# hy-vision-learning/jck-generation

Hardware: AMD Instinct MI355X
Metric: images/sec (G+D step) DCGAN 64x64 bs256 (higher is better)
Workload: dtype bf16; 1 GPU; DCGAN 64x64x3 synthetic, batch 256 per GPU, full G+D step incl. GP pass, RNG and Adam (BASELINE.json configs[1]); per_gpu_batch=256, global_batch=256, parallelism=dp1, dead_D_wgrad_in_G_phase=skipped (never observable: zeroed at train/dcgan_trainer.py:155)

## Files before the change

include/jckgan.h:

```cpp
#ifndef JCKGAN_H
#define JCKGAN_H
#include <stddef.h>
#include <stdint.h>
#ifdef __cplusplus
extern "C" {
#endif

#define JCK_PREC_BF16 0
#define JCK_PREC_F32 1
#define JCK_PREC_BF16X3 2

#define JCK_OK 0
#define JCK_E_ARG (-1)
#define JCK_E_HIP (-2)
#define JCK_E_WS (-3)

const char* jck_last_error(void);
const char* jck_last_launch(void);
const char* jck_launch_name(int i);
int jck_version(void);
int jck_pad_rows(int c);
int jck_pad_chan(int c);

size_t jck_packed_bytes(int prec, long long elems);
// ... 48 lines not shown
                   float* dgamma, float* dbeta, long long rows, int C, void* stream);
int jck_bn_finalize_grouped(const float* stats, int slots_per_group, float count, const float* gamma, const float* beta, float eps,
                            float* aux, float* stat_out, int C, int groups, void* stream);
int jck_bn_fwd(int prec, const void* y, const float* stats, int slots_per_group, float count, const float* gamma, const float* beta,
               float eps, float slope, void* a, float* aux, float* stat_out, float* running_mean, float* running_var, int64_t* nbt,
               float momentum, long long rows_per_group, int C, int groups, void* stream);
int jck_bn_act_fwd_grouped(int prec, const void* y, const float* aux, float slope, void* a, long long rows_per_group, int C,
                           int groups, void* stream);
int jck_bn_act_bwd_grouped(int prec, const void* g_a, const void* y, const float* aux, float slope, float* sums, void* g_y,
                           float* dgamma, float* dbeta, long long rows_per_group, int C, int groups, int grad_groups, void* stream);
size_t jck_grid_sync_bytes(void);
int jck_grid_sync_error(const void* sync_ws);
int jck_bn_act_bwd_res(int prec, const void* g_a, const void* y, const float* aux, float slope, float* sums, void* g_y,
                       float* dgamma, float* dbeta, long long rows_per_group, int C, int groups, int grad_groups, void* sync_ws,
                       void* stream);
int jck_conv_down_grouped(int prec, const void* big, const void* w, void* small_out, float* stats, int* stats_slots, int N, int Hb,
                          int Wb, int Cb, int Cs, int group_images, void* stream);
int jck_conv_up_grouped(int prec, const void* small_in, const void* w, void* big_out, float* stats, int* stats_slots, int N, int Hs,
                        int Ws, int Cs, int Cb, int group_images, void* stream);
int jck_img_prep(int prec, const float* img_nchw, const float* noise_nchw, float keep, float mix, void* out, int N, int HW,
                 void* stream);
int jck_img_prep_u8(int prec, const unsigned char* data, const int64_t* idx, const float* noise, float keep, float mix,
                    void* out_nhwc4, float* out_nchw, int B, int Hs, int Ws, void* stream);
#define JCK_RESIZE_MAX_SRC 1024
#define JCK_RESIZE_TAPS_MAGIC 0x7a736572
long long jck_resize_taps_bytes(int Hs, int Ws, int S);
int jck_resize_taps_build(int Hs, int Ws, int S, void* host_buf);
int jck_img_prep_u8_any(int prec, const unsigned char* data, const int64_t* idx, const unsigned char* flip, const float* noise,
                        const unsigned* rng, int tensor_id, float keep, float mix, void* out_nhwc4, float* out_nchw, int B, int Hs,
                        int Ws, int S, const void* taps_dev, void* stream);
// ... 219 lines not shown
```

jck-generation_amd/csrc/engine.hip:

```cpp
#include <cstdlib>

#include "engine_internal.hpp"
#define JCK_BATCHED_DEFAULT 3

namespace {

constexpr long long ALIGN_F = 64;

void add_param(NetLayout& L, const char* name, int a, int b, int c, int d) {
  TensorInfo ti{name, 0, L.n_params, (long long)a * b * c * d, {a, b, c, d}};
  L.t.push_back(ti);
  L.n_params = (L.n_params + ti.numel + ALIGN_F - 1) / ALIGN_F * ALIGN_F;
}
void add_bn(NetLayout& L, const char* wn, const char* bn, const char* rm, const char* rv, int c) {
  add_param(L, wn, c, 1, 1, 1);
  add_param(L, bn, c, 1, 1, 1);
  TensorInfo m{rm, 1, L.n_bn, c, {c, 1, 1, 1}};
  L.t.push_back(m);
  L.n_bn += (c + ALIGN_F - 1) / ALIGN_F * ALIGN_F;
  TensorInfo v{rv, 2, L.n_bn, c, {c, 1, 1, 1}};
  L.t.push_back(v);
  L.n_bn += (c + ALIGN_F - 1) / ALIGN_F * ALIGN_F;
}

// ... 353 lines not shown
                                    e->P(e->LD, e->dg, "label_embedding.weight"), e->P(e->LD, e->dg, "label_embedding.bias"), B, ws));
  if (side) HIPCHK(hipEventRecord(e->evHead, side));
  return jck_split_rows(e->prec, e->gc, L1_KPAD, TT.FEAT, ga4_out, R3, st);
}

struct XgradEpi { const void* tanh_y; float scale; void* out; hipEvent_t done; bool fused; };
struct DBackward {
  int gw = 1;
  hipStream_t side = nullptr;
  bool join = true, lazy_join = false;
  int part = 0;
  bool resident = true;
  bool xgrad = false;
  XgradEpi* xe = nullptr;
  bool gp_norm = false;
};
static int d_convs_backward(jck_engine* e, const DActs& S, const void* x_in, int B, hipStream_t st, const DBackward& o) {
  const int G = S.groups, gw = o.gw;
  hipStream_t side = gw > 0 ? o.side : nullptr;
  for (int i = TT.NS - 1; i >= 0; --i) {
    const int hb = TT.D_HB[i], cs = TT.D_CS[i], cb = TT.D_CB[i];
    const long long rows = (long long)B * (hb / 2) * (hb / 2);
    const bool resume = o.part == 2 && i == TT.NS - 1;
    const bool split0 = !resume && i == 0 && e->bn_res && e->prec == JCK_PREC_BF16 && gw > 0 && gw < G;
    hipEvent_t done = side && e->ext_events && !resume ? e->evW[i] : nullptr;
    if (!resume)
      JCK_TRY(bn_act_bwd_res_ev(e->prec, S.g[i], S.y[i], S.aux[i], LRELU, S.sums[i], S.g[i], gw ? e->P(e->LD, e->dg, NWN[i]) : nullptr,
                                gw ? e->P(e->LD, e->dg, NBN[i]) : nullptr, rows, cs, split0 ? gw : G, gw,
                                e->bn_res && o.resident ? e->gsync : nullptr, st, done));
    if (!resume && gw) {
      hipStream_t ws;
      JCK_TRY(fork_side(e, i, st, side, &ws, !done));
      JCK_TRY(jck_conv_wgrad(e->prec, S.g[i], i == 0 ? x_in : S.a[i - 1], e->wg_ws, e->wg_ws_bytes, e->P(e->LD, e->dg, CWN[i]), 1, gw * B, hb, hb, cb,
                             cs, ws));
    }
    if (split0) {
      const DActs P = S.group(e, gw, G - gw);
      JCK_TRY(bn_act_bwd_res_ev(e->prec, P.g[i], P.y[i], P.aux[i], LRELU, P.sums[i], P.g[i], nullptr, nullptr, rows, cs, G - gw, 0, e->gsync, st, nullptr));
    }
    if (o.part == 1) {
      HIPCHK(hipEventRecord(e->evTail, side ? side : st));
      e->ss.tail_on_side = side != nullptr;
      if (side && !o.lazy_join) HIPCHK(hipStreamWaitEvent(st, e->evTail, 0));
      return JCK_OK;
    }
    if (i > 0)
      JCK_TRY(jck_conv_up(e->prec, S.g[i], e->d_up[i], S.g[i - 1], nullptr, nullptr, 0, G * B, hb / 2, hb / 2, cs, cb, st));
    else if (o.xgrad) {
      const void* g0 = S.group(e, G - 1, 1).g[0];
      if (o.xe) JCK_TRY(conv_up_tanh_bwd_ev(e->prec, g0, e->d_up[0], o.xe->tanh_y, o.xe->scale, o.xe->out, B, hb / 2, hb / 2, cs, cb, st, o.xe->done, &o.xe->fused));
      if (!o.xe || !o.xe->fused) JCK_TRY(jck_conv_up(e->prec, g0, e->d_up[0], S.gx, nullptr, nullptr, 0, B, hb / 2, hb / 2, cs, cb, st));
    }
  }
  if (o.gp_norm) JCK_TRY(jck_gp_norm(e->prec, S.gx, B, TT.HW, e->acc, 6, e->acc_ld, S.norms, st));
  if (side && o.join) {
    HIPCHK(hipEventRecord(e->evWdone, side));
    if (o.lazy_join) { e->ss.join_pending = true; e->ss.mid_recorded = false; }
    else HIPCHK(hipStreamWaitEvent(st, e->evWdone, 0));
  }
  return JCK_OK;
}
static int d_backward(jck_engine* e, DActs& D, const void* x_in, int B, const float* drop_mask, hipStream_t st, const DBackward& o,
                      bool head_mid_done = false) {
// ... 444 lines not shown
  return jck_engine_repack(e, 1, c.st);
}

static int phase_g_loss(jck_engine* e, const PhaseCtx& c) {
  JCK_TRY(clear_or_memset(e, e->ss.gg_clean_step, c.in->step, c.st, e->gg, e->LG.n_params * sizeof(float)));
  const bool fuse = e->head_fuse;
  JCK_TRY(d_forward(e, c.D0, e->fake, c.B, 3, c.in->drop_mask[3], c.st, !fuse));
  if (fuse && !c.cg) JCK_TRY(d_head(e, c.D0, c.B, 0.9f, 0, 2, 5, c.st, c.D0.g[TT.NS - 1]));
  else if (fuse) {
    const float tg1 = 0.9f;
    const int md1 = 0, sl1 = 2, sp1 = 5;
    JCK_TRY(cg_head_middle(e, c.B, 1, &tg1, &md1, &sl1, &sp1, c.D0.prob, c.D0.ds, c.in->drop_mask[3], c.st));
  } else JCK_TRY(d_head(e, c.D0, c.B, 0.9f, 0, 2, 5, c.st));
  XgradEpi xe = {e->fake_raw, 0.9f, e->g_raw, (c.sA && e->ext_events) ? e->evW[TT.NS - 1] : nullptr, false};
  DBackward bw;
  bw.gw = 0; bw.xgrad = true; bw.xe = e->fuse_tanh ? &xe : nullptr;
  JCK_TRY(d_backward(e, c.D0, e->fake, c.B, c.in->drop_mask[3], c.st, bw, fuse));
  return g_backward(e, c.D0.gx, c.B, c.st, c.sA, xe.fused);
}

static int phase_g_step(jck_engine* e, const PhaseCtx& c) {
  if (!e->hp_holds(c.in->step, c.in->lr) && !e->capturing) JCK_TRY(refresh_adam_scalars(e, c.in->step, c.in->lr, c.st));
  JCK_TRY(adam_net(e, 0, 0, e->LG.n_params, c.in->grad_scale, e->hp2 + 8 * e->parity, c.st, nullptr, e->gema));
  TailJobs t = {};
  for (int i = 0; i < TT.NS; ++i) {
    const int cs = TT.D_CS[i];
    t.l[i].rec = e->d_rs[i] + (size_t)e->parity * 4 * 2 * cs;
    t.l[i].rm = e->dbn + find(e->LD, RMN[i])->offset;
    t.l[i].rv = e->dbn + find(e->LD, RVN[i])->offset;
    t.l[i].nbt = (long long*)(e->dnbt + i);
    t.l[i].C = cs;
// ... 234 lines not shown
```

jck-generation_amd/csrc/ops.hip:

```cpp
#include "ops_internal.hpp"
#include "ew.hpp"
#include "ew_optim.hpp"
#include "latent.hpp"
#include "resize.hpp"

#include <cstdlib>
#include <cstring>
#include <string>

static thread_local std::string g_err;
void jck_set_error(const std::string& s) { g_err = s; }
extern "C" const char* jck_last_error(void) { return g_err.c_str(); }
#ifndef JCK_BUILD_ID
#define JCK_BUILD_ID 100
#endif
extern "C" int jck_version(void) { return JCK_BUILD_ID; }

struct KernelInfo { const char* launch; const char* label; };
#define SAME(s) {s, s}
static constexpr KernelInfo KERNELS[] = {
    SAME("igemm<bf16,128,128>"),   SAME("igemm<bf16,128,64>"),   SAME("igemm<bf16,64,128,img>"),   {nullptr, "igemm<bf16,64,128>"}, SAME("igemm<bf16,16,256>"),
    SAME("igemm<f32,128,128>"),    SAME("igemm<f32,128,64>"),    SAME("igemm<f32,64,128,img>"),    SAME("igemm<f32,64,128>"),       SAME("igemm<f32,16,256>"),
    SAME("igemm<bf16x3,128,128>"), SAME("igemm<bf16x3,128,64>"), SAME("igemm<bf16x3,64,128,img>"), SAME("igemm<bf16x3,64,128>"),    SAME("igemm<bf16x3,16,256>"),
    {"igemm_dma_persist<128,256,8>", "igemm<bf16,128,256>"}, {"igemm_dma_persist<128,128,4>", "igemm<bf16,128,128>"},
    {"igemm_dma_persist<128,64,4>", "igemm<bf16,128,64>"},   {"igemm_dma_persist<64,128,4>", "igemm<bf16,64,128>"},
    {"igemm_dma<128,256,3,ws,8>", "igemm<bf16,128,256>"},    {"igemm_dma<128,128,2>", "igemm<bf16,128,128>"},
    {"igemm_dma<128,64,3,ws>", "igemm<bf16,128,64>"},        {"igemm_dma<64,128,2>", "igemm<bf16,64,128>"},
    {"img_down", "img_down<bf16>"}, {"img_up", "img_up<bf16>"},
    {"wgrad_dma<3,ws>", "wgrad<bf16,128,128>"}, {"wgrad_dma<2>", "wgrad<bf16,128,128>"},
    SAME("wgrad<bf16,128,128>"),   SAME("wgrad<bf16,128,64>"),   SAME("wgrad<bf16,64,64,img>"),   SAME("wgrad<bf16,64,64>"),
    SAME("wgrad<f32,128,128>"),    SAME("wgrad<f32,128,64>"),    SAME("wgrad<f32,64,64,img>"),    SAME("wgrad<f32,64,64>"),
    SAME("wgrad<bf16x3,128,128>"), SAME("wgrad<bf16x3,128,64>"), SAME("wgrad<bf16x3,64,64,img>"), SAME("wgrad<bf16x3,64,64>"),
    {nullptr, "bn_act_fwd"}, {nullptr, "bn_bwd_resident"}, {nullptr, "bn_bwd_3launch"},
    {nullptr, "latent_loss"}, {nullptr, "latent_adam"},
    {nullptr, "conv_up_mask"}, {nullptr, "leaky_affine_bwd"}, {nullptr, "critic_ds"}, {nullptr, "latent_loss_ex"},
    {nullptr, "feat_match"}, {nullptr, "img_prep_u8_any"}};
#undef SAME
static_assert(sizeof(KERNELS) / sizeof(KERNELS[0]) == K_COUNT, "KERNELS and the KernelId offsets disagree");
constexpr bool same_str(const char* a, const char* b) { return *a == *b && (!*a || same_str(a + 1, b + 1)); }
constexpr bool row(KernelId id, const char* launch, const char* label) { return same_str(KERNELS[id].launch, launch) && same_str(KERNELS[id].label, label); }
static_assert(row(kid_igemm<PrecBf16, 128, 128, 1>(), "igemm<bf16,128,128>", "igemm<bf16,128,128>") && row(kid_igemm<PrecBf16, 128, 64, 1>(), "igemm<bf16,128,64>", "igemm<bf16,128,64>") && row(kid_igemm<PrecBf16, 64, 128, 2>(), "igemm<bf16,64,128,img>", "igemm<bf16,64,128,img>") && row(kid_igemm<PrecBf16, 16, 256, 1>(), "igemm<bf16,16,256>", "igemm<bf16,16,256>") &&
              row(kid_igemm<PrecF32, 128, 128, 1>(), "igemm<f32,128,128>", "igemm<f32,128,128>") && row(kid_igemm<PrecF32, 128, 64, 1>(), "igemm<f32,128,64>", "igemm<f32,128,64>") && row(kid_igemm<PrecF32, 64, 128, 2>(), "igemm<f32,64,128,img>", "igemm<f32,64,128,img>") && row(kid_igemm<PrecF32, 64, 128, 1>(), "igemm<f32,64,128>", "igemm<f32,64,128>") && row(kid_igemm<PrecF32, 16, 256, 1>(), "igemm<f32,16,256>", "igemm<f32,16,256>") &&
              row(kid_igemm<PrecBf16x3, 128, 128, 1>(), "igemm<bf16x3,128,128>", "igemm<bf16x3,128,128>") && row(kid_igemm<PrecBf16x3, 128, 64, 1>(), "igemm<bf16x3,128,64>", "igemm<bf16x3,128,64>") && row(kid_igemm<PrecBf16x3, 64, 128, 2>(), "igemm<bf16x3,64,128,img>", "igemm<bf16x3,64,128,img>") && row(kid_igemm<PrecBf16x3, 64, 128, 1>(), "igemm<bf16x3,64,128>", "igemm<bf16x3,64,128>") && row(kid_igemm<PrecBf16x3, 16, 256, 1>(), "igemm<bf16x3,16,256>", "igemm<bf16x3,16,256>") &&
              row(kid_igemm_dma(K_IGEMM_PERSIST, 128, 256), "igemm_dma_persist<128,256,8>", "igemm<bf16,128,256>") && row(kid_igemm_dma(K_IGEMM_PERSIST, 128, 128), "igemm_dma_persist<128,128,4>", "igemm<bf16,128,128>") && row(kid_igemm_dma(K_IGEMM_PERSIST, 128, 64), "igemm_dma_persist<128,64,4>", "igemm<bf16,128,64>") && row(kid_igemm_dma(K_IGEMM_PERSIST, 64, 128), "igemm_dma_persist<64,128,4>", "igemm<bf16,64,128>") &&
              row(kid_igemm_dma(K_IGEMM_DMA, 128, 256), "igemm_dma<128,256,3,ws,8>", "igemm<bf16,128,256>") && row(kid_igemm_dma(K_IGEMM_DMA, 128, 128), "igemm_dma<128,128,2>", "igemm<bf16,128,128>") && row(kid_igemm_dma(K_IGEMM_DMA, 128, 64), "igemm_dma<128,64,3,ws>", "igemm<bf16,128,64>") && row(kid_igemm_dma(K_IGEMM_DMA, 64, 128), "igemm_dma<64,128,2>", "igemm<bf16,64,128>") &&
              row(K_IMG_DOWN, "img_down", "img_down<bf16>") && row(K_IMG_UP, "img_up", "img_up<bf16>") && row(K_WGRAD_DMA_WS, "wgrad_dma<3,ws>", "wgrad<bf16,128,128>") && row(K_WGRAD_DMA, "wgrad_dma<2>", "wgrad<bf16,128,128>") &&
              row(kid_wgrad<PrecBf16, 128, 128, 1>(), "wgrad<bf16,128,128>", "wgrad<bf16,128,128>") && row(kid_wgrad<PrecBf16, 128, 64, 1>(), "wgrad<bf16,128,64>", "wgrad<bf16,128,64>") && row(kid_wgrad<PrecBf16, 64, 64, 2>(), "wgrad<bf16,64,64,img>", "wgrad<bf16,64,64,img>") && row(kid_wgrad<PrecBf16, 64, 64, 1>(), "wgrad<bf16,64,64>", "wgrad<bf16,64,64>") &&
              row(kid_wgrad<PrecF32, 128, 128, 1>(), "wgrad<f32,128,128>", "wgrad<f32,128,128>") && row(kid_wgrad<PrecF32, 128, 64, 1>(), "wgrad<f32,128,64>", "wgrad<f32,128,64>") && row(kid_wgrad<PrecF32, 64, 64, 2>(), "wgrad<f32,64,64,img>", "wgrad<f32,64,64,img>") && row(kid_wgrad<PrecF32, 64, 64, 1>(), "wgrad<f32,64,64>", "wgrad<f32,64,64>") &&
              row(kid_wgrad<PrecBf16x3, 128, 128, 1>(), "wgrad<bf16x3,128,128>", "wgrad<bf16x3,128,128>") && row(kid_wgrad<PrecBf16x3, 128, 64, 1>(), "wgrad<bf16x3,128,64>", "wgrad<bf16x3,128,64>") && row(kid_wgrad<PrecBf16x3, 64, 64, 2>(), "wgrad<bf16x3,64,64,img>", "wgrad<bf16x3,64,64,img>") && row(kid_wgrad<PrecBf16x3, 64, 64, 1>(), "wgrad<bf16x3,64,64>", "wgrad<bf16x3,64,64>") &&
              same_str(KERNELS[K_LATENT_LOSS].label, "latent_loss") && same_str(KERNELS[K_LATENT_ADAM].label, "latent_adam") &&
              same_str(KERNELS[K_CONV_UP_MASK].label, "conv_up_mask") && same_str(KERNELS[K_LEAKY_AFFINE_BWD].label, "leaky_affine_bwd") &&
              same_str(KERNELS[K_CRITIC_DS].label, "critic_ds") && same_str(KERNELS[K_LATENT_LOSS_EX].label, "latent_loss_ex") && same_str(KERNELS[K_FEAT_MATCH].label, "feat_match") && same_str(KERNELS[K_IMG_PREP_ANY].label, "img_prep_u8_any") &&
              same_str(KERNELS[K_BN_ACT_FWD].label, "bn_act_fwd") && same_str(KERNELS[K_BN_BWD_RES].label, "bn_bwd_resident") && same_str(KERNELS[K_BN_BWD_3L].label, "bn_bwd_3launch") &&
              kid_igemm<PrecBf16, 16, 256, 0>() == kid_igemm<PrecBf16, 16, 256, 1>() && !KERNELS[K_IGEMM + 3].launch,
              "KERNELS and the kid_* functions disagree");
static thread_local const char* g_last_launch = "";
void note_launch(KernelId k) { g_last_launch = KERNELS[k].launch ? KERNELS[k].launch : ""; }
extern "C" const char* jck_last_launch(void) { return g_last_launch; }
extern "C" const char* jck_launch_name(int i) {
  for (int k = 0; k < K_COUNT; ++k)
    if (KERNELS[k].launch && i-- == 0) return KERNELS[k].launch;
  return nullptr;
}
extern "C" int jck_pad_rows(int c) { return c <= 16 ? 16 : (c <= 64 ? 64 : (c + 127) / 128 * 128); }
extern "C" int jck_pad_chan(int c) { return c == 3 ? 4 : c; }

static int env_int(const char* name, int dflt) { const char* v = getenv(name); return v ? atoi(v) : dflt; }
// ... 712 lines not shown
```

jck-generation_amd/csrc/ops_bn.hip:

```cpp
#include "ops_internal.hpp"
#include "bn2.hpp"
#include "bnres.hpp"

#include <climits>

static bool bn_channels_ok(int C, int max_c = INT_MAX) { return is_pow2(C) && C >= 8 && C <= max_c; }

constexpr int BN_FUSE_WGS = 256;
static unsigned bn_slice_grid(long long rows, int C, int groups) {
  const long long per = std::max<long long>(1, BN_FUSE_WGS / ((long long)(C / 64) * groups));
  return (unsigned)std::max<long long>(1, std::min<long long>((rows + 31) / 32, per));
}
static bool bn_two_launches(int prec, int C) { return g_bn_bwd_fuse && C >= 64 && C % 64 == 0 && (prec == JCK_PREC_BF16 || g_bn_bwd_fuse > 1); }

extern "C" int jck_bn_finalize(const float* stats, int slots, float count, const float* gamma, const float* beta,
                               float* running_mean, float* running_var, int64_t* nbt, float momentum, float eps, float* aux,
                               int C, void* stream) {
  if (slots < 1) JCK_FAIL(JCK_E_ARG, "bn_finalize: slots must be >= 1");
  if (C % 4) JCK_FAIL(JCK_E_ARG, "bn_finalize: C % 4 != 0");
  hipLaunchKernelGGL(bn_finalize_kernel, dim3(C / 4), dim3(256), 0, (hipStream_t)stream, stats, slots, count, gamma, beta,
                     running_mean, running_var, (long long*)nbt, momentum, eps, aux, C);
  HIPCHK(hipGetLastError());
  return JCK_OK;
}
// ... 185 lines not shown
  const dim3 grid(nb), block(BNRES_THREADS);
  ProfScope prof(K_BN_BWD_RES, 0.0, stream, 3.0 * groups * rows_per_group * C * 2);
  const int ng = (groups >= 3 && 3 * nch <= 16) ? 3 : (groups >= 2 && 2 * nch <= 16) ? 2 : 1;
#define BNRES_CASE(NCH_, NG_) case NCH_ * 4 + NG_: LAUNCH_EV((bn_bwd_res_kernel<NCH_, NG_>), grid, block, 0, stream, done, p); break
  switch (nch * 4 + ng) {
    BNRES_CASE(1, 1); BNRES_CASE(2, 1); BNRES_CASE(4, 1); BNRES_CASE(8, 1); BNRES_CASE(16, 1);
    BNRES_CASE(1, 2); BNRES_CASE(2, 2); BNRES_CASE(4, 2); BNRES_CASE(8, 2);
    BNRES_CASE(1, 3); BNRES_CASE(2, 3); BNRES_CASE(4, 3);
    default: JCK_FAIL(JCK_E_ARG, "bn_act_bwd_res: no kernel for this plan");
  }
#undef BNRES_CASE
  HIPCHK(hipGetLastError());
  return JCK_OK;
}

extern "C" size_t jck_bn2_ws_floats(int C) { return (size_t)(4 + 4 * BN_BWD_MAX_BLOCKS) * C; }
extern "C" int jck_bn2_vchain(int prec, const void* v, const void* y, const void* gy, const float* aux, const float* s1,
                              const float* gamma, float slope, float* ws, void* u, void* xdir, float* dgamma, long long rows, int C,
                              void* stream) {
  if (!bn_channels_ok(C, 2048)) JCK_FAIL(JCK_E_ARG, "bn2_vchain: C must be a power of two in [8, 2048]");
  const int rstep = 256 / (C / 8);
  const int blocks = bn_bwd_blocks(rows, rstep);
  float* partial = ws + 4 * C;
  DISPATCH_T(prec, hipLaunchKernelGGL((bn2_reduce_kernel<T, 1>), dim3(blocks), dim3(256), 3 * C * rstep * sizeof(float),
                                      (hipStream_t)stream, (const T*)v, (const T*)y, (const T*)gy, aux, slope, partial, rows, C));
  HIPCHK(hipGetLastError());
  if (bn_two_launches(prec, C)) {
    DISPATCH_T(prec, hipLaunchKernelGGL(bn2_vchain_apply_fused_kernel<T>, dim3(bn_slice_grid(rows, C, 1), C / 64), dim3(BNF_THREADS), 0,
                                        (hipStream_t)stream, (const T*)v, (const T*)y, (const T*)gy, aux, s1, (const float*)partial, blocks, ws,
                                        gamma, dgamma, slope, 1.0f / (float)rows, (T*)u, (T*)xdir, rows, C));
// ... 42 lines not shown
```

jck-generation_amd/csrc/ops_internal.hpp:

```cpp
#pragma once
#include <hip/hip_ext.h>

#include <algorithm>
#include <cmath>
#include <string>

#include "../../include/jckgan.h"
#include "common.hpp"

void jck_set_error(const std::string& s);

static inline bool prec_f32_storage(int prec) { return prec == JCK_PREC_F32 || prec == JCK_PREC_BF16X3; }
static inline bool is_pow2(int v) { return v > 0 && (v & (v - 1)) == 0; }
static inline unsigned ew_grid(long long n, int per_block = 256) { return (unsigned)std::max<long long>(1, std::min<long long>((n + per_block - 1) / per_block, 8192)); }

#define JCK_FAIL(code, msg)                                   \
  do {                                                        \
    jck_set_error(std::string(__func__) + ": " + (msg));     \
    return (code);                                            \
  } while (0)

#define HIPCHK(expr)                                                                                     \
  do {                                                                                                   \
    hipError_t e_ = (expr);                                                                              \
// ... 25 lines not shown
  K_PRECS = 3,
  K_IGEMM_TILES = 5,
  K_DMA_TILES = 4,
  K_WGRAD_TILES = 4,
  K_IGEMM = 0,
  K_IGEMM_PERSIST = K_IGEMM + K_PRECS * K_IGEMM_TILES,
  K_IGEMM_DMA = K_IGEMM_PERSIST + K_DMA_TILES,
  K_IMG_DOWN = K_IGEMM_DMA + K_DMA_TILES, K_IMG_UP,
  K_WGRAD_DMA_WS, K_WGRAD_DMA,
  K_WGRAD,
  K_BN_ACT_FWD = K_WGRAD + K_PRECS * K_WGRAD_TILES, K_BN_BWD_RES, K_BN_BWD_3L,
  K_LATENT_LOSS, K_LATENT_ADAM,
  K_CONV_UP_MASK, K_LEAKY_AFFINE_BWD, K_CRITIC_DS, K_LATENT_LOSS_EX,
  K_FEAT_MATCH,
  K_IMG_PREP_ANY,
  K_COUNT
};
template <class P> constexpr int kid_prec() { return P::SPLIT ? 2 : P::IS_F32 ? 1 : 0; }
template <class P, int BCH, int BPIX, int NSUB> constexpr KernelId kid_igemm() {
  static_assert(P::IS_F32 || !(BCH == 64 && NSUB == 1), "bf16 has no register-staged 64 x 128 tile (and no name for one)");
  return KernelId(K_IGEMM + K_IGEMM_TILES * kid_prec<P>() + (BCH == 128 ? (BPIX == 128 ? 0 : 1) : BCH == 64 ? (NSUB == 2 ? 2 : 3) : 4));
}
constexpr KernelId kid_igemm_dma(KernelId family, int BCH, int BPIX) { return KernelId(family + (BPIX == 256 ? 0 : BCH == 64 ? 3 : BPIX == 128 ? 1 : 2)); }
template <class P, int BG, int BS, int NSUB> constexpr KernelId kid_wgrad() {
  return KernelId(K_WGRAD + K_WGRAD_TILES * kid_prec<P>() + (BG == 128 ? (BS == 128 ? 0 : 1) : NSUB == 2 ? 2 : 3));
}
void note_launch(KernelId k);

extern bool g_prof_on;
struct ProfRec { KernelId kernel; double flops, bytes; hipStream_t st; hipEvent_t e0, e1; };
// ... 14 lines not shown
                      long long nmask = 0, float keep_p = 0.75f, float* zero = nullptr, long long nzero = 0, float* zbig0 = nullptr,
                      long long nzbig0 = 0, float* zbig1 = nullptr, long long nzbig1 = 0, void* zpad = nullptr, int zd = 0, int zp = 0,
                      int zpad_f32 = 0);
int jck_adam_hp(float* p, const float* g, float* m, float* v, long long n, double beta1, double beta2, double eps,
                float grad_scale, const float* hp, hipStream_t st, float* zero = nullptr, long long nzero = 0,
                const unsigned* skip_if = nullptr,
                float* ema = nullptr);
const unsigned* jck_grid_sync_error_word(const void* sync_ws);
int bn_fwd_fused(int prec, const void* y, const float* stats, int slots_per_group, float count, const float* gamma, const float* beta,
                 float eps, float slope, void* a, float* aux, float* stat_out, float* running_mean, float* running_var, int64_t* nbt,
                 float momentum, long long rows_per_group, int C, int groups, long long out_row, long long out_pitch, hipStream_t stream,
                 bool* fused);
int bn_act_bwd_res_ev(int prec, const void* g_a, const void* y, const float* aux, float slope, float* sums, void* g_y, float* dgamma,
                      float* dbeta, long long rows_per_group, int C, int groups, int grad_groups, void* sync_ws, hipStream_t stream,
                      hipEvent_t done);
int conv_up_tanh_bwd_ev(int prec, const void* small_in, const void* w, const void* tanh_y, float scale, void* out, int N, int Hs, int Ws,
                        int Cs, int Cb, hipStream_t stream, hipEvent_t done, bool* fused);
int head_bwd_conv2_ev(int prec, const float* ds, const float* wp, const void* a4, int B, int B_more, int C, void* g_a4, float* grad, float* ws,
                      hipStream_t stream, hipStream_t side, hipEvent_t handover);
int gp_head2_ev(int prec, const void* ughd, const float* w2, const float* prob, int B, int K, float* rs, float* dw2, float* ws,
                hipStream_t stream, hipStream_t side, hipEvent_t handover);
int pack_linear_pair(int prec, const float* w, int N, int K, int rows0, int cols0, void* wp0, int rows1, int cols1, void* wp1, int permC,
                     int permHW, hipStream_t stream);
int bn_act_fwd_pitched(int prec, const void* y, const float* aux, float slope, void* a, long long rows_per_group, int C, int groups,
                       long long out_row, long long out_pitch, hipStream_t stream);
int cg_head_mid(int prec, const float* slab, int ksplit, const float* bias1, const float* mask, float scale, void* h, void* hd, const float* w2,
                const float* bias2, int B, int G, const float* targets, const int* modes, float* prob, float* ds, float* scal,
                const int* slot_loss, const int* slot_p, int scal_ld, void* g_hd, void* g_h, hipStream_t stream);
int gp_head_mid_ev(int prec, const float* slab, int ksplit, const float* mask, float scale, void* ughd, const float* w2, const float* prob, int B,
                   float* rs, float* dw2, float* ws, void* g_hd, void* g_h, hipStream_t stream, hipStream_t side, hipEvent_t handover);
// ... 5 lines not shown
```

jck-generation_amd/hipgan/_lib.py:

```python
import ctypes as C
import os

import torch

HERE = os.path.dirname(os.path.abspath(__file__))
LIB_PATH = os.path.join(os.path.dirname(HERE), "lib", "libjckgan_hip.so")
PREC_BF16, PREC_F32, PREC_BF16X3 = 0, 1, 2

vp, i32, i64, f32, f64, sz = C.c_void_p, C.c_int, C.c_longlong, C.c_float, C.c_double, C.c_size_t


class StepInputs(C.Structure):
    _fields_ = [("real_nchw", vp), ("noise_real", vp), ("z", vp), ("noise_fake", vp), ("alpha", vp),
                ("lr", f32), ("grad_scale", f32), ("step", i32), ("labels", vp), ("drop_mask", vp * 4),
                ("real_u8", vp), ("real_idx", vp),
                ("real_h", i32), ("real_w", i32), ("real_flip", vp), ("real_taps", vp)]


PROTOS = {
    "jck_last_error": (C.c_char_p, []),
    "jck_last_launch": (C.c_char_p, []),
    "jck_launch_name": (C.c_char_p, [i32]),
    "jck_version": (i32, []),
    "jck_pad_rows": (i32, [i32]),
# ... 27 lines not shown
    "jck_g1_wgrad_ws_bytes": (sz, [i32, i32, i32]),
    "jck_g1_wgrad": (i32, [i32, vp, vp, vp, sz, vp, i32, i32, i32, i32, i32, vp]),
    "jck_bn_finalize": (i32, [vp, i32, f32, vp, vp, vp, vp, vp, f32, f32, vp, i32, vp]),
    "jck_bn_act_fwd": (i32, [i32, vp, vp, f32, vp, i64, i32, vp]),
    "jck_bn_bwd_ws_floats": (sz, [i32]),
    "jck_bn_act_bwd": (i32, [i32, vp, vp, vp, f32, vp, vp, vp, vp, i64, i32, vp]),
    "jck_bn_finalize_grouped": (i32, [vp, i32, f32, vp, vp, f32, vp, vp, i32, i32, vp]),
    "jck_bn_act_fwd_grouped": (i32, [i32, vp, vp, f32, vp, i64, i32, i32, vp]),
    "jck_bn_fwd": (i32, [i32, vp, vp, i32, f32, vp, vp, f32, f32, vp, vp, vp, vp, vp, vp, f32, i64, i32, i32, vp]),
    "jck_conv_down_grouped": (i32, [i32, vp, vp, vp, vp, vp, i32, i32, i32, i32, i32, i32, vp]),
    "jck_conv_up_grouped": (i32, [i32, vp, vp, vp, vp, vp, i32, i32, i32, i32, i32, i32, vp]),
    "jck_bn_act_bwd_grouped": (i32, [i32, vp, vp, vp, f32, vp, vp, vp, vp, i64, i32, i32, i32, vp]),
    "jck_grid_sync_bytes": (sz, []),
    "jck_grid_sync_error": (i32, [vp]),
    "jck_bn_act_bwd_res": (i32, [i32, vp, vp, vp, f32, vp, vp, vp, vp, i64, i32, i32, i32, vp, vp]),
    "jck_img_prep": (i32, [i32, vp, vp, f32, f32, vp, i32, i32, vp]),
    "jck_resize_norm": (i32, [vp, vp, i32, i32, i32, i32, i32, i32, f32, f32, vp, vp, vp]),
    "jck_img_prep_u8": (i32, [i32, vp, vp, vp, f32, f32, vp, vp, i32, i32, i32, vp]),
    "jck_resize_taps_bytes": (i64, [i32, i32, i32]),
    "jck_resize_taps_build": (i32, [i32, i32, i32, vp]),
    "jck_img_prep_u8_any": (i32, [i32, vp, vp, vp, vp, vp, i32, f32, f32, vp, vp, i32, i32, i32, i32, vp, vp]),
    "jck_nhwc4_to_nchw": (i32, [i32, vp, vp, i32, i32, vp]),
    "jck_axpy_noise": (i32, [i32, vp, vp, f32, f32, vp, i32, i32, vp]),
    "jck_interp": (i32, [i32, vp, vp, vp, vp, i32, i32, vp]),
    "jck_mix_interp": (i32, [i32, vp, vp, vp, i32, f32, f32, vp, vp, vp, vp, i32, i32, vp]),
    "jck_gp_norm": (i32, [i32, vp, i32, i32, vp, i32, i32, vp, vp]),
    "jck_tanh_bwd": (i32, [i32, vp, vp, f32, vp, i64, vp]),
    "jck_head_fwd": (i32, [i32, vp, vp, vp, i32, i32, f32, i32, vp, vp, vp, i32, i32, i32, vp]),
    "jck_head_fwd_grouped": (i32, [i32, vp, vp, vp, i32, i32, i32, vp, vp, vp, vp, vp, vp, vp, i32, vp]),
    "jck_head_bwd_ws_floats": (sz, [i32]),
# ... 171 lines not shown
```

Before: 166,400 images/sec.

## Fuse bottom D batchnorm backward with image-gradient conv-up in one resident kernel

Adds a grid-resident kernel that, for the first discriminator layer (32x32x64) during the G phase, computes the BN+LeakyReLU backward per image, does a grid sync for channel statistics, writes the normalized gradient to LDS, and runs the 3x3 transposed conv to the image gradient with MFMA, optionally applying the tanh backward. This replaces the separate bn_act_bwd_res kernel, the global round trip of g_y, and the conv_up/tanh launch. It needs one block per image resident (N <= CU count) and bf16 only, and falls back otherwise. Large LDS and register use per block may limit throughput.

```diff
diff --git a/include/jckgan.h b/include/jckgan.h
--- a/include/jckgan.h
+++ b/include/jckgan.h
@@ -86,6 +86,9 @@
 int jck_bn_act_bwd_res(int prec, const void* g_a, const void* y, const float* aux, float slope, float* sums, void* g_y,
                        float* dgamma, float* dbeta, long long rows_per_group, int C, int groups, int grad_groups, void* sync_ws,
                        void* stream);
+int jck_bn_bwd_img(int prec, const void* g_a, const void* y, const float* aux, float slope, float* sums, float* dgamma, float* dbeta,
+                   const void* w, const void* tanh_y, float scale, void* out, float* scal, int slot, int scal_ld, float* norms, int N,
+                   int Hs, int Ws, int C, void* sync_ws, int* taken, void* stream);
 int jck_conv_down_grouped(int prec, const void* big, const void* w, void* small_out, float* stats, int* stats_slots, int N, int Hb,
                           int Wb, int Cb, int Cs, int group_images, void* stream);
 int jck_conv_up_grouped(int prec, const void* small_in, const void* w, void* big_out, float* stats, int* stats_slots, int N, int Hs,
diff --git a/jck-generation_amd/csrc/bnres_img.hpp b/jck-generation_amd/csrc/bnres_img.hpp
--- /dev/null
+++ b/jck-generation_amd/csrc/bnres_img.hpp
@@ -0,0 +1,240 @@
+#pragma once
+#include "bnres.hpp"
+#include "thin.hpp"
+
+#define BNIMG_HW 32
+#define BNIMG_PIX (BNIMG_HW * BNIMG_HW)
+#define BNIMG_C 64
+#define BNIMG_NCH 16
+#define BNIMG_R 8
+
+struct BnImgParams {
+  const bf16_t* ga; const bf16_t* y;
+  const float* aux;
+  float* sums;
+  unsigned* sync;
+  const bf16_t* w;
+  bf16_t* out;
+  const bf16_t* mul_t; float mul_scale;
+  float* scal; int slot, scal_ld; float* norms; int want_norm;
+  int nb;
+  float slope, inv_count;
+};
+
+__device__ __forceinline__ unsigned bnimg_lds_off(int pixel, int unit) { return (unsigned)(pixel * 128 + ((unit ^ ((pixel >> 1) & 7)) << 4)); }
+
+__global__ __launch_bounds__(BNRES_THREADS) void bn_bwd_img_kernel(const BnImgParams p) {
+  __shared__ __attribute__((aligned(16))) unsigned char sm_img[BNIMG_PIX * BNIMG_C * 2];
+  __shared__ __attribute__((aligned(16))) float sm_wave[8][128];
+  __shared__ __attribute__((aligned(16))) float sm_red[16][128];
+  __shared__ __attribute__((aligned(16))) float sm_cf[5][64];
+  __shared__ float sm_nrm[4];
+  __shared__ int sm_ok;
+  constexpr int C = BNIMG_C, NCH = BNIMG_NCH;
+  const int n = blockIdx.x, nb = p.nb;
+  unsigned gen0 = 0;
+  if (threadIdx.x == 0) {
+    gen0 = bnres_ld(p.sync + BNRES_W_GEN * 32);
+    asm volatile("s_waitcnt vmcnt(0)" ::: "memory");
+  }
+  constexpr unsigned ibytes = BNIMG_PIX * C * 2, kstep = BNRES_ROWS * C * 2;
+  u32x4 vg[NCH], vy[NCH];
+  {
+    const unsigned voff0 = (unsigned)((threadIdx.x >> 3) * C + (threadIdx.x & 7) * 8) * 2u;
+    const auto rg = make_rsrc(p.ga + (long long)n * BNIMG_PIX * C, ibytes);
+    const auto ry = make_rsrc(p.y + (long long)n * BNIMG_PIX * C, ibytes);
+#pragma unroll
+    for (int k = 0; k < NCH; ++k) {
+      vg[k] = __builtin_amdgcn_raw_buffer_load_b128(rg, (int)(voff0 + kstep * k), 0, 2);
+      vy[k] = __builtin_amdgcn_raw_buffer_load_b128(ry, (int)(voff0 + kstep * k), 0, 2);
+    }
+  }
+  int t = threadIdx.x;
+  asm volatile("" : "+v"(t));
+  const int u = t & 7, lane = t & 63, wave = t >> 6;
+  {
+    const int c0 = u * 8;
+    float sc[8], sh[8], mu[8];
+    {
+      const f32x4 a0 = *reinterpret_cast<const f32x4*>(p.aux + c0), a1 = *reinterpret_cast<const f32x4*>(p.aux + c0 + 4);
+      const f32x4 b0 = *reinterpret_cast<const f32x4*>(p.aux + C + c0), b1 = *reinterpret_cast<const f32x4*>(p.aux + C + c0 + 4);
+      const f32x4 m0 = *reinterpret_cast<const f32x4*>(p.aux + 2 * C + c0), m1 = *reinterpret_cast<const f32x4*>(p.aux + 2 * C + c0 + 4);
+#pragma unroll
+      for (int i = 0; i < 4; ++i) { sc[i] = a0[i]; sc[4 + i] = a1[i]; sh[i] = b0[i]; sh[4 + i] = b1[i]; mu[i] = m0[i]; mu[4 + i] = m1[i]; }
+    }
+    float s1[8], s2[8];
+#pragma unroll
+    for (int i = 0; i < 8; ++i) { s1[i] = 0.f; s2[i] = 0.f; }
+#pragma unroll
+    for (int k = 0; k < NCH; ++k) {
+#pragma unroll
+      for (int i = 0; i < 4; ++i) asm volatile("" : "+v"(vg[k][i]), "+v"(vy[k][i]));
+#pragma unroll
+      for (int i = 0; i < 4; ++i) {
+        const float y0 = bnres_lo(vy[k][i]), y1 = bnres_hi(vy[k][i]), q0 = bnres_lo(vg[k][i]), q1 = bnres_hi(vg[k][i]);
+        const float z0 = y0 * sc[2 * i] + sh[2 * i], z1 = y1 * sc[2 * i + 1] + sh[2 * i + 1];
+        const float gz0 = z0 > 0.f ? q0 : p.slope * q0, gz1 = z1 > 0.f ? q1 : p.slope * q1;
+        s1[2 * i] += gz0; s1[2 * i + 1] += gz1;
+        s2[2 * i] += gz0 * (y0 - mu[2 * i]); s2[2 * i + 1] += gz1 * (y1 - mu[2 * i + 1]);
+      }
+#pragma unroll
+      for (int i = 0; i < 8; ++i) asm volatile("" : "+v"(s1[i]), "+v"(s2[i]));
+      __builtin_amdgcn_sched_barrier(0);
+    }
+#pragma unroll
+    for (int i = 0; i < 8; ++i) {
+#pragma unroll
+      for (int o = 8; o < 64; o <<= 1) { s1[i] += __shfl_xor(s1[i], o, 64); s2[i] += __shfl_xor(s2[i], o, 64); }
+    }
+    if (lane < 8) {
+#pragma unroll
+      for (int i = 0; i < 8; ++i) { sm_wave[wave][lane * 8 + i] = s1[i]; sm_wave[wave][64 + lane * 8 + i] = s2[i]; }
+    }
+  }
+  __syncthreads();
+  if (t < 128) {
+    float* prow = p.sums + 2 * C + (long long)n * 128;
+    float v = 0.f;
+#pragma unroll
+    for (int w = 0; w < 8; ++w) v += sm_wave[w][t];
+    __hip_atomic_store(prow + t, v, __ATOMIC_RELAXED, __HIP_MEMORY_SCOPE_AGENT);
+  }
+  asm volatile("s_waitcnt vmcnt(0)" ::: "memory");
+  bnres_grid_sync(p.sync, gen0 + 1u, nb, &sm_ok);
+  {
+    const int q = t & 31, rl = t >> 5;
+    const float* base = p.sums + 2 * C + q * 4;
+    f32x4 acc = {0.f, 0.f, 0.f, 0.f};
+    for (int r = rl; r < nb; r += 64) {
+      f32x4 v[4];
+#pragma unroll
+      for (int e = 0; e < 4; ++e) {
+        v[e] = f32x4{0.f, 0.f, 0.f, 0.f};
+        if (r + 16 * e < nb) v[e] = *reinterpret_cast<const f32x4*>(base + (long long)(r + 16 * e) * 128);
+      }
+#pragma unroll
+      for (int e = 0; e < 4; ++e) acc += v[e];
+    }
+    *reinterpret_cast<f32x4*>(&sm_red[rl][q * 4]) = acc;
+  }
+  __syncthreads();
+  if (t < 128) {
+    float v = 0.f;
+#pragma unroll
+    for (int r = 0; r < 16; ++r) v += sm_red[r][t];
+    sm_wave[0][t] = v;
+  }
+  __syncthreads();
+  if (t < 64) {
+    const float is = p.aux[3 * C + t];
+    const float t1 = sm_wave[0][t], t2 = sm_wave[0][64 + t] * is;
+    sm_cf[0][t] = p.aux[t]; sm_cf[1][t] = p.aux[C + t]; sm_cf[2][t] = p.aux[2 * C + t];
+    sm_cf[3][t] = t1 * p.inv_count; sm_cf[4][t] = is * (t2 * p.inv_count);
+    if (n == 0) { p.sums[t] = t1; p.sums[C + t] = t2; }
+  }
+  __syncthreads();
+  {
+    float sc[8], sh[8], mu[8], m1[8], k2[8];
+#pragma unroll
+    for (int i = 0; i < 8; ++i) {
+      sc[i] = sm_cf[0][u * 8 + i]; sh[i] = sm_cf[1][u * 8 + i]; mu[i] = sm_cf[2][u * 8 + i];
+      m1[i] = sm_cf[3][u * 8 + i]; k2[i] = sm_cf[4][u * 8 + i];
+    }
+    unsigned char* dst = sm_img + bnimg_lds_off(t >> 3, u);
+#pragma unroll
+    for (int k = 0; k < NCH; ++k) {
+      u32x4 o;
+#pragma unroll
+      for (int i = 0; i < 4; ++i) asm volatile("" : "+v"(vg[k][i]), "+v"(vy[k][i]));
+#pragma unroll
+      for (int i = 0; i < 4; ++i) {
+        const float y0 = bnres_lo(vy[k][i]), y1 = bnres_hi(vy[k][i]), q0 = bnres_lo(vg[k][i]), q1 = bnres_hi(vg[k][i]);
+        const float z0 = y0 * sc[2 * i] + sh[2 * i], z1 = y1 * sc[2 * i + 1] + sh[2 * i + 1];
+        const float gz0 = z0 > 0.f ? q0 : p.slope * q0, gz1 = z1 > 0.f ? q1 : p.slope * q1;
+        const float r0 = sc[2 * i] * (gz0 - m1[2 * i] - (y0 - mu[2 * i]) * k2[2 * i]);
+        const float r1 = sc[2 * i + 1] * (gz1 - m1[2 * i + 1] - (y1 - mu[2 * i + 1]) * k2[2 * i + 1]);
+        o[i] = pack2bf_pk(r0, r1);
+      }
+      *reinterpret_cast<u32x4*>(dst + k * kstep) = o;
+      __builtin_amdgcn_sched_barrier(0);
+    }
+  }
+  asm volatile("" ::: "memory");
+  const int pcol = lane & 15, g = lane >> 4;
+  bf16x8 wf[18];
+#pragma unroll
+  for (int f = 0; f < 18; ++f) wf[f] = *reinterpret_cast<const bf16x8*>(p.w + pcol * 576 + f * 32 + g * 8);
+  const int x0 = (wave & 1) << 4, y0 = (wave >> 1) * BNIMG_R, x = x0 + pcol;
+  u32x2 mt[BNIMG_R] = {};
+  if (p.mul_t) {
+#pragma unroll
+    for (int i = 0; i < BNIMG_R; ++i)
+      mt[i] = *reinterpret_cast<const u32x2*>(p.mul_t + (((long long)n * 2 * BNIMG_HW + 2 * (y0 + i) + (g >> 1)) * 2 * BNIMG_HW + 2 * x + (g & 1)) * 4);
+  }
+  __syncthreads();
+  {
+    const int xh = pcol == 0 ? x0 - 1 : (pcol == 15 ? x0 + 16 : -1);
+    const bool okh = (unsigned)xh < (unsigned)BNIMG_HW;
+    struct Row { u32x4 c[2], l[2], r[2]; };
+    auto shift_in = [&](int yy, Row& w) {
+      const bool oky = (unsigned)yy < (unsigned)BNIMG_HW;
+#pragma unroll
+      for (int h = 0; h < 2; ++h) {
+        u32x4 c = {0u, 0u, 0u, 0u}, e = {0u, 0u, 0u, 0u};
+        if (oky) {
+          c = *reinterpret_cast<const u32x4*>(sm_img + bnimg_lds_off(yy * BNIMG_HW + x, g + 4 * h));
+          if (okh) e = *reinterpret_cast<const u32x4*>(sm_img + bnimg_lds_off(yy * BNIMG_HW + xh, g + 4 * h));
+        }
+        w.c[h] = c;
+        w.l[h] = dpp_from_left(e, c);
+        w.r[h] = dpp_from_right(e, c);
+      }
+    };
+    Row win[3];
+    shift_in(y0 - 1, win[0]);
+    shift_in(y0, win[1]);
+#pragma unroll
+    for (int i = 0; i < BNIMG_R; ++i) {
+      shift_in(y0 + i + 1, win[(i + 2) % 3]);
+      f32x4 acc = {0.f, 0.f, 0.f, 0.f};
+#pragma unroll
+      for (int d = 0; d < 3; ++d) {
+        const Row& w = win[(i + d) % 3];
+#pragma unroll
+        for (int h = 0; h < 2; ++h) {
+          acc = mfma16(wf[(d * 3 + 0) * 2 + h], __builtin_bit_cast(bf16x8, w.l[h]), acc);
+          acc = mfma16(wf[(d * 3 + 1) * 2 + h], __builtin_bit_cast(bf16x8, w.c[h]), acc);
+          acc = mfma16(wf[(d * 3 + 2) * 2 + h], __builtin_bit_cast(bf16x8, w.r[h]), acc);
+        }
+      }
+      float v[4] = {acc[0], acc[1], acc[2], acc[3]};
+      const int y = y0 + i;
+      const long long o = (((long long)n * 2 * BNIMG_HW + 2 * y + (g >> 1)) * 2 * BNIMG_HW + 2 * x + (g & 1)) * 4;
+      if (p.mul_t) {
+        const float tt[4] = {bnres_lo(mt[i][0]), bnres_hi(mt[i][0]), bnres_lo(mt[i][1]), bnres_hi(mt[i][1])};
+#pragma unroll
+        for (int r = 0; r < 4; ++r) v[r] = p.mul_scale * bf2f(f2bf(v[r])) * (1.f - tt[r] * tt[r]);
+      }
+      st4(p.out + o, v);
+    }
+  }
+  if (!p.want_norm) return;
+  __syncthreads();
+  float s = 0.f;
+  if (t < 256) {
+    const bf16_t* q = p.out + (long long)n * (4 * BNIMG_PIX) * 4;
+    for (int i = t; i < 4 * BNIMG_PIX; i += 256) {
+      float v[4];
+      ld4(q + i * 4, v);
+      s += v[0] * v[0] + v[1] * v[1] + v[2] * v[2] + v[3] * v[3];
+    }
+    s = wave_sum(s);
+    if (lane == 0) sm_nrm[wave] = s;
+  }
+  __syncthreads();
+  if (t == 0) {
+    const float nr = sqrtf(sm_nrm[0] + sm_nrm[1] + sm_nrm[2] + sm_nrm[3]);
+    if (p.norms) p.norms[n] = nr;
+    if (p.scal && p.slot >= 0) p.scal[(long long)p.slot * p.scal_ld + n] = (nr - 1.f) * (nr - 1.f);
+  }
+}
diff --git a/jck-generation_amd/csrc/engine.hip b/jck-generation_amd/csrc/engine.hip
--- a/jck-generation_amd/csrc/engine.hip
+++ b/jck-generation_amd/csrc/engine.hip
@@ -391,7 +391,18 @@
   bool xgrad = false;
   XgradEpi* xe = nullptr;
   bool gp_norm = false;
+  bool gy_dead = false;
 };
+static int d_bottom_fused(jck_engine* e, const DActs& S, int B, hipStream_t st, const DBackward& o, bool* taken) {
+  const int hb = TT.D_HB[0], cs = TT.D_CS[0], cb = TT.D_CB[0];
+  *taken = false;
+  if (!o.gy_dead || !o.xgrad || o.gp_norm || o.gw || S.groups != 1 || !e->bn_res || !o.resident || jck_pad_chan(cb) != 4) return JCK_OK;
+  JCK_TRY(bn_bwd_img_ev(e->prec, S.g[0], S.y[0], S.aux[0], LRELU, S.sums[0], nullptr, nullptr, e->d_up[0], o.xe ? o.xe->tanh_y : nullptr,
+                        o.xe ? o.xe->scale : 1.f, o.xe ? o.xe->out : S.gx, nullptr, -1, 0, nullptr, B, hb / 2, hb / 2, cs, e->gsync, st,
+                        o.xe ? o.xe->done : nullptr, taken));
+  if (*taken && o.xe) o.xe->fused = true;
+  return JCK_OK;
+}
 static int d_convs_backward(jck_engine* e, const DActs& S, const void* x_in, int B, hipStream_t st, const DBackward& o) {
   const int G = S.groups, gw = o.gw;
   hipStream_t side = gw > 0 ? o.side : nullptr;
@@ -401,7 +412,9 @@
     const bool resume = o.part == 2 && i == TT.NS - 1;
     const bool split0 = !resume && i == 0 && e->bn_res && e->prec == JCK_PREC_BF16 && gw > 0 && gw < G;
     hipEvent_t done = side && e->ext_events && !resume ? e->evW[i] : nullptr;
-    if (!resume)
+    bool img = false;
+    if (!resume && i == 0) JCK_TRY(d_bottom_fused(e, S, B, st, o, &img));
+    if (!resume && !img)
       JCK_TRY(bn_act_bwd_res_ev(e->prec, S.g[i], S.y[i], S.aux[i], LRELU, S.sums[i], S.g[i], gw ? e->P(e->LD, e->dg, NWN[i]) : nullptr,
                                 gw ? e->P(e->LD, e->dg, NBN[i]) : nullptr, rows, cs, split0 ? gw : G, gw,
                                 e->bn_res && o.resident ? e->gsync : nullptr, st, done));
@@ -423,7 +436,7 @@
     }
     if (i > 0)
       JCK_TRY(jck_conv_up(e->prec, S.g[i], e->d_up[i], S.g[i - 1], nullptr, nullptr, 0, G * B, hb / 2, hb / 2, cs, cb, st));
-    else if (o.xgrad) {
+    else if (o.xgrad && !img) {
       const void* g0 = S.group(e, G - 1, 1).g[0];
       if (o.xe) JCK_TRY(conv_up_tanh_bwd_ev(e->prec, g0, e->d_up[0], o.xe->tanh_y, o.xe->scale, o.xe->out, B, hb / 2, hb / 2, cs, cb, st, o.xe->done, &o.xe->fused));
       if (!o.xe || !o.xe->fused) JCK_TRY(jck_conv_up(e->prec, g0, e->d_up[0], S.gx, nullptr, nullptr, 0, B, hb / 2, hb / 2, cs, cb, st));
@@ -898,7 +911,7 @@
   } else JCK_TRY(d_head(e, c.D0, c.B, 0.9f, 0, 2, 5, c.st));
   XgradEpi xe = {e->fake_raw, 0.9f, e->g_raw, (c.sA && e->ext_events) ? e->evW[TT.NS - 1] : nullptr, false};
   DBackward bw;
-  bw.gw = 0; bw.xgrad = true; bw.xe = e->fuse_tanh ? &xe : nullptr;
+  bw.gw = 0; bw.xgrad = true; bw.xe = e->fuse_tanh ? &xe : nullptr; bw.gy_dead = true;
   JCK_TRY(d_backward(e, c.D0, e->fake, c.B, c.in->drop_mask[3], c.st, bw, fuse));
   return g_backward(e, c.D0.gx, c.B, c.st, c.sA, xe.fused);
 }
diff --git a/jck-generation_amd/csrc/ops.hip b/jck-generation_amd/csrc/ops.hip
--- a/jck-generation_amd/csrc/ops.hip
+++ b/jck-generation_amd/csrc/ops.hip
@@ -34,7 +34,7 @@
     {nullptr, "bn_act_fwd"}, {nullptr, "bn_bwd_resident"}, {nullptr, "bn_bwd_3launch"},
     {nullptr, "latent_loss"}, {nullptr, "latent_adam"},
     {nullptr, "conv_up_mask"}, {nullptr, "leaky_affine_bwd"}, {nullptr, "critic_ds"}, {nullptr, "latent_loss_ex"},
-    {nullptr, "feat_match"}, {nullptr, "img_prep_u8_any"}};
+    {nullptr, "feat_match"}, {nullptr, "img_prep_u8_any"}, {nullptr, "bn_bwd_img"}};
 #undef SAME
 static_assert(sizeof(KERNELS) / sizeof(KERNELS[0]) == K_COUNT, "KERNELS and the KernelId offsets disagree");
 constexpr bool same_str(const char* a, const char* b) { return *a == *b && (!*a || same_str(a + 1, b + 1)); }
@@ -50,7 +50,7 @@
               row(kid_wgrad<PrecBf16x3, 128, 128, 1>(), "wgrad<bf16x3,128,128>", "wgrad<bf16x3,128,128>") && row(kid_wgrad<PrecBf16x3, 128, 64, 1>(), "wgrad<bf16x3,128,64>", "wgrad<bf16x3,128,64>") && row(kid_wgrad<PrecBf16x3, 64, 64, 2>(), "wgrad<bf16x3,64,64,img>", "wgrad<bf16x3,64,64,img>") && row(kid_wgrad<PrecBf16x3, 64, 64, 1>(), "wgrad<bf16x3,64,64>", "wgrad<bf16x3,64,64>") &&
               same_str(KERNELS[K_LATENT_LOSS].label, "latent_loss") && same_str(KERNELS[K_LATENT_ADAM].label, "latent_adam") &&
               same_str(KERNELS[K_CONV_UP_MASK].label, "conv_up_mask") && same_str(KERNELS[K_LEAKY_AFFINE_BWD].label, "leaky_affine_bwd") &&
-              same_str(KERNELS[K_CRITIC_DS].label, "critic_ds") && same_str(KERNELS[K_LATENT_LOSS_EX].label, "latent_loss_ex") && same_str(KERNELS[K_FEAT_MATCH].label, "feat_match") && same_str(KERNELS[K_IMG_PREP_ANY].label, "img_prep_u8_any") &&
+              same_str(KERNELS[K_CRITIC_DS].label, "critic_ds") && same_str(KERNELS[K_LATENT_LOSS_EX].label, "latent_loss_ex") && same_str(KERNELS[K_FEAT_MATCH].label, "feat_match") && same_str(KERNELS[K_IMG_PREP_ANY].label, "img_prep_u8_any") && same_str(KERNELS[K_BN_BWD_IMG].label, "bn_bwd_img") &&
               same_str(KERNELS[K_BN_ACT_FWD].label, "bn_act_fwd") && same_str(KERNELS[K_BN_BWD_RES].label, "bn_bwd_resident") && same_str(KERNELS[K_BN_BWD_3L].label, "bn_bwd_3launch") &&
               kid_igemm<PrecBf16, 16, 256, 0>() == kid_igemm<PrecBf16, 16, 256, 1>() && !KERNELS[K_IGEMM + 3].launch,
               "KERNELS and the kid_* functions disagree");
diff --git a/jck-generation_amd/csrc/ops_bn.hip b/jck-generation_amd/csrc/ops_bn.hip
--- a/jck-generation_amd/csrc/ops_bn.hip
+++ b/jck-generation_amd/csrc/ops_bn.hip
@@ -1,6 +1,7 @@
 #include "ops_internal.hpp"
 #include "bn2.hpp"
 #include "bnres.hpp"
+#include "bnres_img.hpp"
 
 #include <climits>
 
@@ -223,6 +224,36 @@
   return JCK_OK;
 }
 
+int bn_bwd_img_ev(int prec, const void* g_a, const void* y, const float* aux, float slope, float* sums, float* dgamma, float* dbeta,
+                  const void* w, const void* tanh_y, float scale, void* out, float* scal, int slot, int scal_ld, float* norms, int N, int Hs,
+                  int Ws, int C, void* sync_ws, hipStream_t stream, hipEvent_t done, bool* taken) {
+  *taken = g_bn_res && sync_ws && prec == JCK_PREC_BF16 && C == BNIMG_C && Hs == BNIMG_HW && Ws == BNIMG_HW && !dgamma && !dbeta &&
+           N >= 1 && N <= bnres_cus() && N <= BN_BWD_MAX_BLOCKS;
+  if (!*taken) return JCK_OK;
+  if (!g_a || !y || !aux || !sums || !w || !out) JCK_FAIL(JCK_E_ARG, "bn_bwd_img: null tensor");
+  const bool want_norm = norms || (scal && slot >= 0);
+  if (scal && slot >= 0 && scal_ld < N) JCK_FAIL(JCK_E_ARG, "bn_bwd_img: scal_ld < N");
+  BnImgParams p;
+  p.ga = (const bf16_t*)g_a; p.y = (const bf16_t*)y; p.aux = aux; p.sums = sums; p.sync = (unsigned*)sync_ws;
+  p.w = (const bf16_t*)w; p.out = (bf16_t*)out; p.mul_t = (const bf16_t*)tanh_y; p.mul_scale = scale;
+  p.scal = scal; p.slot = slot; p.scal_ld = scal_ld; p.norms = norms; p.want_norm = want_norm ? 1 : 0;
+  p.nb = N; p.slope = slope; p.inv_count = 1.0f / (float)((long long)N * BNIMG_PIX);
+  ProfScope prof(K_BN_BWD_IMG, 0.0, stream, 2.0 * N * BNIMG_PIX * C * 2 + 4.0 * N * BNIMG_PIX * 4 * 2);
+  LAUNCH_EV(bn_bwd_img_kernel, dim3(N), dim3(BNRES_THREADS), 0, stream, done, p);
+  HIPCHK(hipGetLastError());
+  return JCK_OK;
+}
+extern "C" int jck_bn_bwd_img(int prec, const void* g_a, const void* y, const float* aux, float slope, float* sums, float* dgamma,
+                              float* dbeta, const void* w, const void* tanh_y, float scale, void* out, float* scal, int slot, int scal_ld,
+                              float* norms, int N, int Hs, int Ws, int C, void* sync_ws, int* taken, void* stream) {
+  bool t = false;
+  if (!taken) JCK_FAIL(JCK_E_ARG, "bn_bwd_img: taken is required");
+  const int rc = bn_bwd_img_ev(prec, g_a, y, aux, slope, sums, dgamma, dbeta, w, tanh_y, scale, out, scal, slot, scal_ld, norms, N, Hs, Ws,
+                               C, sync_ws, (hipStream_t)stream, nullptr, &t);
+  *taken = t ? 1 : 0;
+  return rc;
+}
+
 extern "C" size_t jck_bn2_ws_floats(int C) { return (size_t)(4 + 4 * BN_BWD_MAX_BLOCKS) * C; }
 extern "C" int jck_bn2_vchain(int prec, const void* v, const void* y, const void* gy, const float* aux, const float* s1,
                               const float* gamma, float slope, float* ws, void* u, void* xdir, float* dgamma, long long rows, int C,
diff --git a/jck-generation_amd/csrc/ops_internal.hpp b/jck-generation_amd/csrc/ops_internal.hpp
--- a/jck-generation_amd/csrc/ops_internal.hpp
+++ b/jck-generation_amd/csrc/ops_internal.hpp
@@ -63,6 +63,7 @@
   K_CONV_UP_MASK, K_LEAKY_AFFINE_BWD, K_CRITIC_DS, K_LATENT_LOSS_EX,
   K_FEAT_MATCH,
   K_IMG_PREP_ANY,
+  K_BN_BWD_IMG,
   K_COUNT
 };
 template <class P> constexpr int kid_prec() { return P::SPLIT ? 2 : P::IS_F32 ? 1 : 0; }
@@ -107,6 +108,9 @@
 int bn_act_bwd_res_ev(int prec, const void* g_a, const void* y, const float* aux, float slope, float* sums, void* g_y, float* dgamma,
                       float* dbeta, long long rows_per_group, int C, int groups, int grad_groups, void* sync_ws, hipStream_t stream,
                       hipEvent_t done);
+int bn_bwd_img_ev(int prec, const void* g_a, const void* y, const float* aux, float slope, float* sums, float* dgamma, float* dbeta,
+                  const void* w, const void* tanh_y, float scale, void* out, float* scal, int slot, int scal_ld, float* norms, int N, int Hs,
+                  int Ws, int C, void* sync_ws, hipStream_t stream, hipEvent_t done, bool* taken);
 int conv_up_tanh_bwd_ev(int prec, const void* small_in, const void* w, const void* tanh_y, float scale, void* out, int N, int Hs, int Ws,
                         int Cs, int Cb, hipStream_t stream, hipEvent_t done, bool* fused);
 int head_bwd_conv2_ev(int prec, const float* ds, const float* wp, const void* a4, int B, int B_more, int C, void* g_a4, float* grad, float* ws,
diff --git a/jck-generation_amd/hipgan/_lib.py b/jck-generation_amd/hipgan/_lib.py
--- a/jck-generation_amd/hipgan/_lib.py
+++ b/jck-generation_amd/hipgan/_lib.py
@@ -65,6 +65,7 @@
     "jck_grid_sync_bytes": (sz, []),
     "jck_grid_sync_error": (i32, [vp]),
     "jck_bn_act_bwd_res": (i32, [i32, vp, vp, vp, f32, vp, vp, vp, vp, i64, i32, i32, i32, vp, vp]),
+    "jck_bn_bwd_img": (i32, [i32, vp, vp, vp, f32, vp, vp, vp, vp, vp, f32, vp, vp, i32, i32, vp, i32, i32, i32, i32, vp, C.POINTER(i32), vp]),
     "jck_img_prep": (i32, [i32, vp, vp, f32, f32, vp, i32, i32, vp]),
     "jck_resize_norm": (i32, [vp, vp, i32, i32, i32, i32, i32, i32, f32, f32, vp, vp, vp]),
     "jck_img_prep_u8": (i32, [i32, vp, vp, vp, f32, f32, vp, vp, i32, i32, i32, vp]),
```

Measured after the change: 167,500 images/sec (median of 6 runs). No clear change (+0.7%).
